# XinArkh/VNect

Measured on AMD Instinct MI355X. Metric: frames/sec, 368x368 3-scale VNect inference, higher is better.
Workload: dtype f32

## Files before the change

include/vnect_abi.h:

```cpp
#ifndef VNECT_ABI_H
#define VNECT_ABI_H
#include <stdint.h>
#ifdef __cplusplus
extern "C" {
#endif

#define VNECT_ABI_VERSION 7
#define VNECT_MAX_SCALES 8
#define VNECT_MAX_STREAMS 4
#define VNECT_BOX 368
#define VNECT_HM 46
#define VNECT_JOINTS 21

enum {
    VNECT_OK = 0,
    VNECT_E_ARG = -1,
    VNECT_E_STATE = -2,
    VNECT_E_HIP = -3,
    VNECT_E_NODEVICE = -4,
    VNECT_E_TIMESTAMP = -5,
    VNECT_E_COMM = -6,
    VNECT_E_TIMEORDER = -7,
    VNECT_E_INTERNAL = -8
};
// ... 197 lines not shown
    double total_ms;
    double net_ms;
    double conv_ms;
    int32_t conv_launches;
    double conv_flops;
    double conv_slot_ms;
    double shader_cycles;
    double shader_ticks;
} vnect_timings;
int vnect_set_profiling(vnect_handle* h, int on);
int vnect_get_timings(vnect_handle* h, vnect_timings* out);
int vnect_reset_timings(vnect_handle* h);

typedef struct vnect_layer_info {
    char name[64];
    int32_t M, N, K;
    int32_t tile_m, tile_n, split_k, workgroups;
    double flops;
    double last_ms;
} vnect_layer_info;
int vnect_get_layer_info(vnect_handle* h, int idx, vnect_layer_info* out);
int vnect_get_batch_layer_info(vnect_handle* h, int idx, vnect_layer_info* out);
int vnect_get_layer_rows(vnect_handle* h, int idx, int batch, int32_t* rows_computed, int32_t* live_rule_stride);
int vnect_get_layer_stamps(vnect_handle* h, int idx, uint64_t* out24);

int vnect_comm_unique_id(void* id128);
int vnect_comm_init(vnect_handle* h, int rank, int nranks, const void* id128);
int vnect_comm_library(char* path_out, int capacity, int32_t* reused_out);
int vnect_comm_p2p_export(vnect_handle* h, void* blob128);
int vnect_comm_p2p_init(vnect_handle* h, int rank, int nranks, const void* blobs);

#ifdef __cplusplus
}
#endif
#endif
```

vnect_amd/_native.py:

```python
import ctypes as C
import os
import subprocess

import numpy as np

_HERE = os.path.dirname(os.path.abspath(__file__))
LIB_PATH = os.environ.get("VNECT_LIB") or os.path.join(_HERE, "lib", "libvnect_hip.so")
_lib = None

MAX_SCALES = 8
OK, E_ARG, E_STATE, E_HIP, E_NODEVICE, E_TIMESTAMP, E_COMM, E_TIMEORDER, E_INTERNAL = 0, -1, -2, -3, -4, -5, -6, -7, -8
ABI_VERSION = 7
MAX_STREAMS = 4
XCHG_RCCL, XCHG_P2P = 0, 1
FP32, BF16, FP32_SPLIT, FP16 = 0, 1, 2, 3


class VnectError(RuntimeError):
    def __init__(self, code, msg):
        super().__init__("libvnect_hip: %s (code %d)" % (msg, code))
        self.code = code


class Config(C.Structure):
# ... 165 lines not shown
    "vnect_forward": (C.c_int, [_H, _f32p, C.c_int, _f32p]),
    "vnect_preprocess": (C.c_int, [_H, _u8p, C.c_int, C.c_int, C.c_int64, _f32p, _f64p, _i32p, _i32p]),
    "vnect_postprocess": (C.c_int, [_H, _f32p, C.c_double, C.c_double, C.c_double, C.c_int32, C.c_int32, _f64p, _f32p]),
    "vnect_infer": (C.c_int, [_H, _u8p, C.c_int, C.c_int, C.c_int64, C.c_double, C.c_double, _f64p, _f32p]),
    "vnect_frame_buffer": (C.c_int, [_H, C.c_int, C.c_int64, C.POINTER(_u8p)]),
    "vnect_upload_frame": (C.c_int, [_H, C.c_int, _u8p, C.c_int, C.c_int, C.c_int64]),
    "vnect_infer_resident": (C.c_int, [_H, C.c_int, C.c_double, C.c_double, _f64p, _f32p]),
    "vnect_submit_resident": (C.c_int, [_H, C.c_int, C.c_double, C.c_double]),
    "vnect_collect": (C.c_int, [_H, _f64p, _f32p]),
    "vnect_submit_stream": (C.c_int, [_H, C.c_int, C.c_int, C.c_double, C.c_double]),
    "vnect_collect_stream": (C.c_int, [_H, _i32p, _f64p, _f32p]),
    "vnect_reset_filters_stream": (C.c_int, [_H, C.c_int]),
    "vnect_set_stream_batch": (C.c_int, [_H, C.c_int]),
    "vnect_submit_streams": (C.c_int, [_H, C.c_int, _i32p, _i32p, _f64p, _f64p]),
    "vnect_get_batch_layer_info": (C.c_int, [_H, C.c_int, C.POINTER(LayerInfo)]),
    "vnect_joint_filter": (C.c_int, [_H, C.c_int, _f64p, C.c_int, C.c_double, _f64p]),
    "vnect_reset_filters": (C.c_int, [_H]),
    "vnect_read_activation": (C.c_int, [_H, C.c_char_p, _f32p, C.c_int64, _i32p]),
    "vnect_set_profiling": (C.c_int, [_H, C.c_int]),
    "vnect_get_timings": (C.c_int, [_H, C.POINTER(Timings)]),
    "vnect_reset_timings": (C.c_int, [_H]),
    "vnect_get_layer_info": (C.c_int, [_H, C.c_int, C.POINTER(LayerInfo)]),
    "vnect_get_layer_rows": (C.c_int, [_H, C.c_int, C.c_int, C.POINTER(C.c_int32), C.POINTER(C.c_int32)]),
    "vnect_get_layer_stamps": (C.c_int, [_H, C.c_int, C.POINTER(C.c_uint64)]),
    "vnect_comm_unique_id": (C.c_int, [C.c_void_p]),
    "vnect_comm_init": (C.c_int, [_H, C.c_int, C.c_int, C.c_void_p]),
    "vnect_comm_library": (C.c_int, [C.c_char_p, C.c_int, _i32p]),
    "vnect_comm_p2p_export": (C.c_int, [_H, C.c_void_p]),
    "vnect_comm_p2p_init": (C.c_int, [_H, C.c_int, C.c_int, C.c_void_p]),
    "vnect_track_begin": (C.c_int, [_H, C.c_int, C.c_int, C.c_int, _i32p]),
    "vnect_submit_tracked": (C.c_int, [_H, C.c_int, C.c_int, C.c_double, C.c_double]),
    "vnect_submit_tracked_pinned": (C.c_int, [_H, C.c_int, C.c_int, C.c_int64, C.c_double, C.c_double]),
    "vnect_collect_tracked": (C.c_int, [_H, _i32p, _f64p, _f32p, _i32p]),
    "vnect_track_box": (C.c_int, [_H, C.c_int, _i32p]),
    "vnect_result_confidence": (C.c_int, [_H, _f64p, _i32p]),
    "vnect_track_policy": (C.c_int, [_H, C.c_int, C.c_double, C.c_int, C.c_int]),
    "vnect_upload_frame_nv12": (C.c_int, [_H, C.c_int, _u8p, C.c_int64, _u8p, C.c_int64, C.c_int, C.c_int]),
    "vnect_upload_frame_nv12_rect": (C.c_int, [_H, C.c_int, _u8p, C.c_int64, _u8p, C.c_int64, C.c_int, C.c_int, _i32p]),
    "vnect_infer_nv12": (C.c_int, [_H, _u8p, C.c_int64, _u8p, C.c_int64, C.c_int, C.c_int, _i32p, C.c_double, C.c_double, _f64p, _f32p]),
    "vnect_preprocess_nv12": (C.c_int, [_H, _u8p, C.c_int64, _u8p, C.c_int64, C.c_int, C.c_int, _i32p, _f32p, _f64p, _i32p, _i32p]),
    "vnect_submit_tracked_pinned_nv12": (C.c_int, [_H, C.c_int, C.c_int, C.c_int64, C.c_int64, C.c_int64, C.c_double, C.c_double]),
    "vnect_read_frame": (C.c_int, [_H, C.c_int, _u8p, C.c_int64, _i32p]),
    "vnect_upload_frame_device": (C.c_int, [_H, C.c_int, C.POINTER(DeviceFrame), C.c_void_p]),
    "vnect_infer_device": (C.c_int, [_H, C.POINTER(DeviceFrame), C.c_void_p, C.c_double, C.c_double, _f64p, _f32p]),
    "vnect_preprocess_device": (C.c_int, [_H, C.POINTER(DeviceFrame), C.c_void_p, _f32p, _f64p, _i32p, _i32p]),
    "vnect_submit_tracked_device": (C.c_int, [_H, C.c_int, C.POINTER(DeviceFrame), C.c_void_p, C.c_double, C.c_double]),
# ... 546 lines not shown
    def reset_timings(self):
        self._ck(lib().vnect_reset_timings(self._h))

    def layer_stamps(self, idx):
        buf = (C.c_uint64 * 24)()
        self._ck(lib().vnect_get_layer_stamps(self._h, idx, buf))
        return list(buf)

    def layers(self):
        return self._layer_list(lib().vnect_get_layer_info)

    def layer_rows(self, batch=False):
        out, i = [], 0
        while True:
            rows, rule = C.c_int32(), C.c_int32()
            rc = lib().vnect_get_layer_rows(self._h, i, int(batch), C.byref(rows), C.byref(rule))
            if rc == E_STATE:
                self._ck(rc)
            if rc:
                return out
            out.append((rows.value, rule.value))
            i += 1

    def _layer_list(self, fn):
        out, i = [], 0
        while True:
            li = LayerInfo()
            rc = fn(self._h, i, C.byref(li))
            if rc == E_STATE:
                self._ck(rc)
            if rc:
                return out
            out.append({k: (getattr(li, k).decode() if k == "name" else getattr(li, k)) for k, _ in LayerInfo._fields_})
            i += 1


def _as_frame(img):
    img = np.asarray(img)
    if img.dtype != np.uint8 or img.ndim != 3 or img.shape[2] != 3:
        raise ValueError("frame must be a uint8 (H, W, 3) BGR array")
    if img.strides[2] != 1 or img.strides[1] != 3 or img.strides[0] < img.shape[1] * 3:
        img = np.ascontiguousarray(img)
    return img


def _as_nv12(nv12):
# ... 134 lines not shown
```

vnect_amd/csrc/conv.hip:

```cpp
#include "kernels.h"

#ifndef X3_DBG
#define X3_DBG 0
#endif
#ifndef VNECT_AB
#define VNECT_AB 0
#endif
#ifndef BF16_NOSTORE
#define BF16_NOSTORE 0
#endif

#include <array>
#include <cstddef>
#include <cstdlib>
#include <type_traits>
#include <utility>

namespace vnect {

typedef float f32x16 __attribute__((ext_vector_type(16)));
typedef float f32x4 __attribute__((ext_vector_type(4)));
typedef __bf16 bf16x8 __attribute__((ext_vector_type(8)));
typedef __bf16 bf16x4 __attribute__((ext_vector_type(4)));
typedef _Float16 f16x8 __attribute__((ext_vector_type(8)));
// ... 58 lines not shown
    *(__attribute__((address_space(1))) h16<BF>*)p = b;
#else
    __hip_atomic_store((unsigned short*)p, __builtin_bit_cast(unsigned short, b), __ATOMIC_RELAXED, __HIP_MEMORY_SCOPE_AGENT);
#endif
}

#if defined(__HIP_DEVICE_COMPILE__)
typedef __amdgpu_buffer_rsrc_t srd_t;
__device__ __forceinline__ srd_t make_srd(const void* base)
{
    return __builtin_amdgcn_make_buffer_rsrc((void*)base, 0, 0x7fffffff, 0x00020000);
}
__device__ __forceinline__ void bload_lds(srd_t r, float* lds, unsigned voff, unsigned soff)
{
    __builtin_amdgcn_raw_ptr_buffer_load_lds(r, (__attribute__((address_space(3))) void*)lds, 16, (int)voff, (int)soff, 0, 0);
}
#else
typedef int srd_t;
__device__ __forceinline__ srd_t make_srd(const void*) { return 0; }
__device__ __forceinline__ void bload_lds(srd_t, float*, unsigned, unsigned) {}
#endif

typedef __attribute__((address_space(3))) unsigned lds_u32;
__device__ __forceinline__ void live_fill(const ConvArgs& a, int M, int Wo, int Ho, unsigned mg_wo, unsigned mg_ho, int m0, int lane, lds_u32* tab)
{
    const int m = m0 + lane;
    const bool ok = m < M;
    const int mm = ok ? m : 0;
    const int t = fdiv(mm, mg_wo, Wo), ox = mm - t * Wo;
    const int sI = fdiv(t, mg_ho, Ho), oy = t - sI * Ho;
    const int pix = (sI * a.OH + oy * a.os) * a.OW + ox * a.os;
    tab[lane] = ok ? (unsigned)(pix * a.ldc) * 4u : 0x80000000u;
}
#if defined(__HIP_DEVICE_COMPILE__)
__device__ __forceinline__ unsigned bload_u32(srd_t r, unsigned voff, unsigned soff) { return __builtin_amdgcn_raw_buffer_load_b32(r, (int)voff, (int)soff, 0); }
__device__ __forceinline__ void bstore_f32(srd_t r, float v, unsigned voff, unsigned soff)
{
    __builtin_amdgcn_raw_buffer_store_b32(__builtin_bit_cast(unsigned, v), r, (int)voff, (int)soff, 16);
}
#else
__device__ __forceinline__ unsigned bload_u32(srd_t, unsigned, unsigned) { return 0; }
__device__ __forceinline__ void bstore_f32(srd_t, float, unsigned, unsigned) {}
#endif
__device__ __forceinline__ void live_load_resid(srd_t rs, const lds_u32* tab, int rb, int cb, int lane, unsigned (&rw)[16])
{
    const unsigned colb = (unsigned)((lane & 31) * 4);
    const lds_u32* lt = tab + rb;
    asm volatile("" ::: "memory");
#pragma unroll
    for (int r = 0; r < 16; r++) rw[r] = bload_u32(rs, lt[(r & 3) + 8 * (r >> 2)] + colb, (unsigned)(cb * 128));
}

constexpr int BONE_N0 = 128, BONE_LS = 68;
__device__ __forceinline__ float bone_len(float x, float y, float z)
{
// ... 559 lines not shown
        auto item_A = [&](const Item& it) __attribute__((always_inline)) {
            tb = __builtin_amdgcn_readfirstlane(it.phase * h.ntaps);
            if constexpr (SPAN) {
                const SpanGeo g = span_geo(it.m0);
                const int slot = wave * 64 + lane;
                const int grow = slot < g.c0 ? g.t0 : g.t0 + 1;
                const int xp = slot < g.c0 ? 2 * g.ox0 + slot : slot - g.c0;
                const int sI = fdiv(grow, h.mg_ho, h.Ho), oy = grow - sI * h.Ho;
                const bool live = slot < g.c0 + g.c1 && grow * h.Wo < h.M;
                a_vo[0] = 0, a_mask[0] = 0;
#pragma unroll
                for (int i = 1; i < ARB; i++) a_vo[i] = 0, a_mask[i] = 0;
                if (live) {
                    const int iy = oy * p.stride, ix = xp;
                    a_vo[0] = (unsigned)(((sI * p.H + iy) * p.W + ix) * p.Cs * ESZ);
                    for (int t2 = 0; t2 < h.ntaps; t2++) {
                        const int y = iy + tap_dy(tb + t2), x = ix + tap_dx(tb + t2);
                        a_mask[0] |= ((unsigned)y < (unsigned)p.H && (unsigned)x < (unsigned)p.W ? 1u : 0u) << t2;
                    }
                }
            }
#pragma unroll
            for (int i = 0; i < (SPAN ? 0 : ARB); i++) {
                const int mraw = it.m0 + srow + 32 * i;
                const bool live = mraw < h.M;
                const int m = live ? mraw : 0;
                const int t = fdiv(m, h.mg_wo, h.Wo), ox = m - t * h.Wo;
                const int s = fdiv(t, h.mg_ho, h.Ho), oy = t - s * h.Ho;
                const int iy = oy * p.stride + (pix && BF ? unit >> 2 : 0);
                const int ix = ox * p.stride + (pix ? (BF ? (unit & 3) * 2 : unit) : 0);
                a_vo[i] = live ? (unsigned)(((s * p.H + iy) * p.W + ix) * p.Cs * ESZ + (pix ? 0 : unit * 16)) : 0u;
                const unsigned vx = (ix >= 1 ? 1u : 0u) | 2u | (ix + 1 < p.W ? 4u : 0u);
                const unsigned m3 = (iy >= 1 ? vx : 0u) | (vx << 3) | (iy + 1 < p.H ? vx << 6 : 0u);
                unsigned mk = a.tapgrid == 1 ? 1u : m3;
                if (a.tapgrid == 0) {
                    mk = 0;
                    for (int t2 = 0; t2 < h.ntaps; t2++) {
                        const int y = iy + tap_dy(tb + t2), x = ix + tap_dx(tb + t2);
                        mk |= ((unsigned)y < (unsigned)p.H && (unsigned)x < (unsigned)p.W ? 1u : 0u) << t2;
                    }
                }
                a_mask[i] = live ? mk : 0u;
            }
            tap = __builtin_amdgcn_readfirstlane(fdiv(it.c0, p.mg_cpt, h.cpt)), cc = __builtin_amdgcn_readfirstlane(it.c0 - tap * h.cpt);
            rem = __builtin_amdgcn_readfirstlane(it.cnt);
            set_tap(tap);
        };
        auto item_B = [&](const Item& it) __attribute__((always_inline)) {
// ... 62 lines not shown
            loads(stage, std::true_type{}, std::true_type{}, 0u);
            advance();
        };
        auto wait_landed = [&](int young) __attribute__((always_inline)) {
            switch (young) {
                case 1: wait_vm<NLD>(); break;
                case 2: wait_vm<2 * NLD>(); break;
                case 3: wait_vm<3 * NLD>(); break;
                case 4: wait_vm<4 * NLD>(); break;
                case 5: wait_vm<5 * NLD>(); break;
                case 6: wait_vm<6 * NLD>(); break;
                case 7: wait_vm<7 * NLD>(); break;
                default: wait_vm<0>(); break;
            }
        };
        TailRegs<BF> T;
        WideRegs<BF> TW;
        const int wm2 = wave & 1, g2 = wave >> 1;
        if constexpr (TAIL && WIDE) wide_load_weights<BF>(a, wave, lane, TW), wide_load_resid<BF>(a, decode(0).m0, wave, lane, TW);
        lds_u32* const ltab = (lds_u32*)smem + (NS - 1) * STAGE + (4 + wave) * 64;
        const bool live = LIVE && a.os != 1;
        if constexpr (TAIL && !WIDE) {
            const int mb2 = decode(0).m0 + wm2 * 32 + 4 * (lane >> 5);
            if (live) {
                if constexpr (LIVE) {
                    live_fill(a, h.M, h.Wo, h.Ho, h.mg_wo, h.mg_ho, decode(0).m0, lane, ltab);
                    const srd_t srdR = make_srd(a.resid);
                    live_load_resid(srdR, ltab, wm2 * 32 + 4 * (lane >> 5), 2 + g2, lane, T.rw[0]);
                    live_load_resid(srdR, ltab, wm2 * 32 + 4 * (lane >> 5), 4 + g2, lane, T.rw[1]);
                }
            } else {
                tail_load_resid<BF>(a, mb2, 2 + g2, lane, T.rw[0]);
                tail_load_resid<BF>(a, mb2, 4 + g2, lane, T.rw[1]);
            }
            tail_load_b<BF>(a, 2 + g2, lane, T.Bf);
        }
        const bool pst = P2 && threadIdx.x == 256 && blockIdx.x == 0;
        if (pst) prof[22] = __builtin_amdgcn_s_memrealtime();
        int nis = 0, istage = 0, g = 0;
        auto put = [&]() __attribute__((always_inline)) {
            issue(istage);
            istage = istage + 1 == NS ? 0 : istage + 1, nis++;
        };
        constexpr bool BFIRST = SINGLE && !X3;
        if constexpr (BFIRST) {
            const Item it = decode(0);
            item_B(it);
            loads(0, std::false_type{}, std::true_type{}, 0u);
            if (G > 1) loads(1, std::false_type{}, std::true_type{}, STEP_B);
            item_A(it);
            if (pst) prof[23] = __builtin_amdgcn_s_memrealtime();
            loads(0, std::true_type{}, std::false_type{}, 0u);
            advance();
            if (G > 1) {
                loads(1, std::true_type{}, std::false_type{}, 0u);
                advance();
            }
            nis = G > 1 ? 2 : 1, istage = nis;
// ... 26 lines not shown
            pw += q1 - q0, pb += q2 - q1, pi += q3 - q2;
        }
        if (pacct) prof[16] = pw, prof[17] = pb, prof[18] = pi;
        if constexpr (TAIL) {
            __builtin_amdgcn_s_barrier();
            if constexpr (WIDE) {
                f32x4 Cq[CHAIN_DEPTH<BF>];
                tail_wide<BF, CHAIN>(a, smem, decode(0).m0, wave, lane, TW, Cq);
                if constexpr (CHAIN) {
                    asm volatile("s_waitcnt lgkmcnt(0)" ::: "memory");
                    __builtin_amdgcn_s_barrier();
                    if constexpr (BF) {
                        if (wide_staged<BF>(a)) wide_write_out(a, smem, decode(0).m0);
                    }
                    chain_gemm<BF>(a, smem, decode(0).m0, wave, lane, Cq);
                } else if constexpr (BF) {
                    if (wide_staged<BF>(a)) {
                        asm volatile("s_waitcnt lgkmcnt(0)" ::: "memory");
                        __builtin_amdgcn_s_barrier();
                        wide_write_out(a, smem, decode(0).m0);
                    }
                }
            } else {
                bool live2 = false;
                if constexpr (LIVE) {
                    int os2;
                    asm volatile("s_load_dword %0, %1, %2\n\ts_waitcnt lgkmcnt(0)" : "=s"(os2) : "s"(__builtin_amdgcn_kernarg_segment_ptr()), "n"(offsetof(ConvArgs, os)) : "memory");
                    live2 = os2 != 1;
                }
                if (live2) live_fill(a, h.M, h.Wo, h.Ho, h.mg_wo, h.mg_ho, decode(0).m0, lane, ltab);
                tail_gemm<BF, 3, true, CHAIN>(a, smem, decode(0).m0, wm2, 2 + g2, 2, lane, T, live2 ? ltab : nullptr);
                if constexpr (CHAIN) chain_narrow<BF>(a, smem, decode(0).m0, wave, lane);
                else if constexpr (BF) {
                    if (tail_staged<BF>(a)) {
                        asm volatile("s_waitcnt lgkmcnt(0)" ::: "memory");
                        __builtin_amdgcn_s_barrier();
                        tail_write_out(a, smem, decode(0).m0);
                    }
                }
            }
        }
        if constexpr (BONE) {
            const Item it0 = decode(0);
            if (it0.n0 <= BONE_N0 && it0.n0 + BN > BONE_N0) {
                __builtin_amdgcn_s_barrier();
                bone_features<BF>(a, smem, it0.m0, it0.phase, tid, h.M, h.Wo, h.Ho, h.mg_wo, h.mg_ho);
            }
        }
        return;
    }

    int fo[4];
#pragma unroll
    for (int q = 0; q < 4; q++) fo[q] = (lane & 31) * 32 + (((2 * q + (lane >> 5)) ^ ((lane >> 1) & 7)) * 4);
// ... 365 lines not shown
                asm volatile("s_waitcnt lgkmcnt(0)" ::: "memory");
                __builtin_amdgcn_s_barrier();
            }
            if constexpr (WIDE) {
                tail_wide<BF, CHAIN>(a, smem, it.m0, 4 + wave, lane, TWc);
                if constexpr (CHAIN) {
                    asm volatile("s_waitcnt lgkmcnt(0)" ::: "memory");
                    __builtin_amdgcn_s_barrier();
                    if constexpr (BF) {
                        if (wide_staged<BF>(a)) wide_write_out(a, smem, it.m0);
                    }
                } else if constexpr (BF) {
                    if (wide_staged<BF>(a)) {
                        asm volatile("s_waitcnt lgkmcnt(0)" ::: "memory");
                        __builtin_amdgcn_s_barrier();
                        wide_write_out(a, smem, it.m0);
                    }
                }
            } else {
                TailRegs<BF> T;
                lds_u32* const ltab = (lds_u32*)smem + (NS - 1) * STAGE + wave * 64;
                const bool live = LIVE && c.os != 1;
                if (live) live_fill(a, h.M, h.Wo, h.Ho, h.mg_wo, h.mg_ho, it.m0, lane, ltab);
                tail_gemm<BF, 1, false, CHAIN>(a, smem, it.m0, wm2, g2, 0, lane, T, live ? ltab : nullptr);
                if constexpr (CHAIN) {
                    asm volatile("s_waitcnt lgkmcnt(0)" ::: "memory");
                    __builtin_amdgcn_s_barrier();
                    tail_write_out(a, smem, it.m0);
                } else if constexpr (BF) {
                    if (tail_staged<BF>(a)) {
                        asm volatile("s_waitcnt lgkmcnt(0)" ::: "memory");
                        __builtin_amdgcn_s_barrier();
                        tail_write_out(a, smem, it.m0);
                    }
                }
            }
            break;
        }
        if constexpr (NACC > 1) {
            asm volatile("s_waitcnt vmcnt(0)" : "+v"(bias), "+v"(sc), "+v"(sh), "+v"(biasx[0]), "+v"(scx[0]), "+v"(shx[0]), "+v"(biasx[NACC - 2]), "+v"(scx[NACC - 2]), "+v"(shx[NACC - 2]));
            const int py = it.phase >> 1, px = it.phase & 1;
            gfloat* const outp = (gfloat*)c.out;
            bool relub[NACC];
#pragma unroll
            for (int b = 0; b < NACC; b++) relub[b] = it.n0 + (wn + b) * 32 < c.relu_cols;
#pragma unroll
            for (int r = 0; r < 16; r++) {
// ... 230 lines not shown
constexpr StreamKernel stream_kernel_at()
{
    constexpr Variant v = variant_at(I);
    static_assert(variant_index(v) == I, "variant_at is the inverse of variant_index: slot I holds the kernel the launcher looks up there");
    if constexpr (variant_exists<BM, BN, KG>(v))
        return {conv_stream_kernel<BM, BN, KG, ring_depth<BM, BN, KG>(v.x3), v.el, v.prof, v.fuse, v.span, v.x3, v.one>, variant_lds<BM, BN, KG>(v.x3)};
    else
        return {nullptr, 0};
}
template <int BM, int BN, int KG, int... I>
constexpr std::array<StreamKernel, sizeof...(I)> stream_kernels(std::integer_sequence<int, I...>)
{
    return {{stream_kernel_at<BM, BN, KG, I>()...}};
}
template <int BM, int BN, int KG>
constexpr auto STREAM_KERNELS = stream_kernels<BM, BN, KG>(std::make_integer_sequence<int, N_VARIANTS>{});

template <int BM, int BN, int KG>
static hipError_t launch_stream(ConvArgs a, hipStream_t st)
{
    if (a.cpt % KG != 0 || a.Npad % BN != 0) return hipErrorInvalidValue;
    a.cpt /= KG;
    int live_grid = 0;
    if (a.live_s != 0) {
        const bool form = BM == 64 && BN == 64 && KG == 1 && a.tail_n == 256 && !a.bf16 && !a.x3 && a.chain_n == 0 && !a.bone;
        if (!form || a.live_s < 2 || !a.resid || a.ldr != a.ldc || a.Nvalid != a.tail_n || a.stride != 1 || a.os != 1 || a.nphase != 1 || a.ksplit != 1 ||
            a.tapgrid != 3 || a.OH != a.Ho || a.OW != a.Wo || a.H != a.Ho || a.W != a.Wo)
            return hipErrorInvalidValue;
        live_grid = ((a.M + BM - 1) / BM) * (a.Npad / BN);
        a.stride = a.os = a.live_s;
        a.Ho = (a.Ho + a.live_s - 1) / a.live_s, a.Wo = (a.Wo + a.live_s - 1) / a.live_s;
        a.M = a.S * a.Ho * a.Wo;
    }
    a.tiles_m = (a.M + BM - 1) / BM, a.tiles_n = a.Npad / BN;
    auto magic = [](int d) { return (unsigned)((0x100000000ull + (unsigned)d - 1) / (unsigned)d); };
    a.mg_wo = magic(a.Wo), a.mg_ho = magic(a.Ho), a.mg_tn = magic(a.tiles_n), a.mg_tm = magic(a.tiles_m);
    a.mg_ks = magic(a.ksplit), a.mg_cpt = magic(a.cpt);
    a.items = a.tiles_m * a.tiles_n * a.nphase * a.ksplit;
    static const int maxwg_env = getenv("VNECT_MAXWG") ? atoi(getenv("VNECT_MAXWG")) : 0;
    const int cus = g_cus;
    const int maxwg = maxwg_env > 0 ? maxwg_env : (KG == 1 && BN <= 64 ? 2 * cus : cus);
    static const bool no_one = getenv("VNECT_NO_ONE") != nullptr, no_big = getenv("VNECT_NO_BIG_GRID") != nullptr;
    const bool plain64 = KG == 1 && BN <= 64 && maxwg_env <= 0 && !no_big && !a.x3 && !a.pixmode;
    const bool big_grid = plain64 && (a.bf16 ? a.items <= 4 * cus : (a.ntaps * a.cpt <= 8 && a.items <= 8 * cus));
    const bool one = a.ksplit == 1 && !no_one && (a.items <= maxwg || big_grid);
    const bool fused = a.tail_n > 0 || a.bone;
    dim3 grid(live_grid ? live_grid : (one || fused) ? a.items : (a.items < maxwg ? a.items : maxwg));
    static const bool detail = getenv("VNECT_PROF_DETAIL") && atoi(getenv("VNECT_PROF_DETAIL")) != 0;
    const int prof = a.prof ? (detail ? 2 : 1) : 0;

    if (a.x3) {
        if (a.bf16 || a.pixmode || a.K % 32) return hipErrorInvalidValue;
        if (a.chain_n != 0) return hipErrorInvalidValue;
    }
    if (a.tail_n > 0) {
        if (a.bone || a.ksplit != 1 || a.nphase != 1 || (a.os != 1 && !live_grid) || !a.tail_w || !a.tail_bias) return hipErrorInvalidValue;
        if constexpr (BN == 128) {
            if (a.Npad != 128 || a.tail_n > 512 ||
                (a.chain_n != 0 && (a.chain_n != 128 || a.tail_n != 512 || !a.chain_w || !a.chain_bias || !a.chain_out || a.chain_ld < 128)))
                return hipErrorInvalidValue;
        } else {
            if (a.Npad != 64 || a.tail_n != 256) return hipErrorInvalidValue;
            if (a.chain_n != 0 && (!a.bf16 || a.chain_n != 64 || !a.chain_w || !a.chain_bias || !a.chain_out || a.chain_ld < 64 || !a.resid ||
                                   a.relu_cols < 256 || a.out_f32 || a.Nvalid != 256 ||
                                   (a.ldc & 7) != 0))
                return hipErrorInvalidValue;
        }
    }
    if (a.bone && (a.ksplit != 1 || a.Npad != 192 || a.ldc < 212)) return hipErrorInvalidValue;
    if constexpr (BN == 96) {
        if (a.bf16 || a.x3 || a.tail_n > 0 || a.resid || a.out2 || a.ksplit != 1 || a.pixmode || (a.relu_cols & 31)) return hipErrorInvalidValue;
    }

    Variant v{};
    v.el = a.f16 ? EL_F16 : a.bf16 ? EL_BF16 : EL_F32;
    v.fuse = a.tail_n > 0 ? (a.chain_n ? 3 : 1) : a.bone ? 2 : 0;
    v.x3 = a.x3 != 0;
    v.span = variant_exists<BM, BN, KG>({EL_F32, 0, 0, true, false, false}) && !v.x3 && v.fuse == 0 && a.pixmode && !a.bf16 && a.ksplit == 1 &&
             a.cpt == 1 && a.Wo >= 64 && a.stride == 2 && getenv("VNECT_NO_SPAN") == nullptr;
// ... 188 lines not shown
```

vnect_amd/csrc/hostplan.h:

```cpp
#pragma once
#include <math.h>
#include <stdint.h>
#include <stdio.h>
#include <stdlib.h>
#include <string.h>

#include <algorithm>
#include <string>
#include <utility>
#include <vector>

#include "axis.h"
#include "tables.h"

namespace vnect {
namespace plan {

inline int cv_round(double v) { return (int)nearbyint(v); }
inline int clipi(int x, int a, int b) { return x >= a ? (x < b ? x : b - 1) : a; }
inline int16_t sat_short(float v)
{
    int r = (int)nearbyintf(v);
    return (int16_t)(r < -32768 ? -32768 : (r > 32767 ? 32767 : r));
}
// ... 408 lines not shown

struct LiveNode {
    int in, resid, out, out2, out3;
    int ntaps, stride;
    int tap00;
    int tail;
};
inline int live_rows_stride(const LiveNode* L, int n, int li, int t_final)
{
    if (li < 0 || li >= n || !L[li].tail || L[li].out < 0 || L[li].out3 >= 0) return 0;
    const int t = L[li].out;
    if (t == t_final) return 0;
    int s = 0;
    for (int j = 0; j < n; j++) {
        if (j == li) continue;
        if (L[j].resid == t) return 0;
        if (L[j].out == t || L[j].out2 == t || L[j].out3 == t) return 0;
        if (L[j].in != t) continue;
        if (L[j].ntaps != 1 || !L[j].tap00 || L[j].stride < 2 || (s && L[j].stride != s)) return 0;
        s = L[j].stride;
    }
    return s;
}
inline int live_dim(int n, int s) { return (n + s - 1) / s; }
inline int live_rows(int S, int Ho, int Wo, int s) { return S * live_dim(Ho, s) * live_dim(Wo, s); }
inline void live_enumeration(int S, int Ho, int Wo, int s, std::vector<int>& pix)
{
    const int Hl = live_dim(Ho, s), Wl = live_dim(Wo, s);
    pix.clear();
    pix.reserve((size_t)S * Ho * Wo);
    for (int j = 0; j < S * Hl * Wl; j++) {
        const int ox = j % Wl, t = j / Wl, oy = t % Hl, im = t / Hl;
        pix.push_back((im * Ho + oy * s) * Wo + ox * s);
    }
    for (int p = 0; p < S * Ho * Wo; p++)
        if ((p % Wo) % s != 0 || ((p / Wo) % Ho) % s != 0) pix.push_back(p);
}
inline int live_wg_tile(int tiles, int grid, int id)
{
    if (id < 0 || id >= grid) return -1;
    const int xcd = id & 7, l = id >> 3, qd = tiles >> 3, rm = tiles & 7;
    const int lo = xcd < rm ? xcd * (qd + 1) : rm * (qd + 1) + (xcd - rm) * qd, cnt = qd + (xcd < rm ? 1 : 0);
    return l < cnt ? lo + l : -1;
}

}
}
```

vnect_amd/csrc/hostplan_capi.cpp:

```cpp
#include <stdint.h>
#include <string.h>

#include <vector>

#include "axis.h"
#include "crop.h"
#include "hostplan.h"

using namespace vnect;

extern "C" {

int hp_resize_u8(const uint8_t* src, int sh, int sw, int ch, double f, uint8_t* dst, int* dh, int* dw)
{
    std::vector<ResizeTab> t(1);
    if (!plan::build_u8_tab(sh, sw, f, &t[0])) return -1;
    *dh = t[0].dh, *dw = t[0].dw;
    if (!dst) return 0;
    for (int y = 0; y < t[0].dh; y++)
        for (int x = 0; x < t[0].dw; x++)
            for (int c = 0; c < ch; c++)
                dst[((size_t)y * t[0].dw + x) * ch + c] =
                    (uint8_t)plan::sample_u8([&](int r, int q) { return (int)src[((size_t)r * sw + q) * ch + c]; }, t[0], y, x);
    return 0;
// ... 248 lines not shown
    memcpy(out, &fp[0], sizeof(FrameParams));
    return status;
}
const char* hp_crop_refusal(int code) { return crop_refusal(code); }
void hp_box_update(const double* j2, int n, int W, int H, int fallback, int32_t* rects)
{
    for (int i = 0; i < n; i++) {
        int r[4];
        box_update(j2 + (size_t)i * NJ * 2, W, H, r);
        if (fallback) box_fallback(W, H, r);
        for (int k = 0; k < 4; k++) rects[(size_t)i * 4 + k] = r[k];
    }
}

int hp_live_rows_stride(const int32_t* nodes, int n, int li, int t_final)
{
    std::vector<plan::LiveNode> L(n > 0 ? n : 0);
    for (int i = 0; i < n; i++) {
        const int32_t* q = nodes + (size_t)i * 9;
        L[i] = {q[0], q[1], q[2], q[3], q[4], q[5], q[6], q[7], q[8]};
    }
    return plan::live_rows_stride(L.data(), n, li, t_final);
}
int hp_live_rows(int S, int Ho, int Wo, int s) { return plan::live_rows(S, Ho, Wo, s); }
void hp_live_enumeration(int S, int Ho, int Wo, int s, int32_t* pix)
{
    std::vector<int> v;
    plan::live_enumeration(S, Ho, Wo, s, v);
    for (size_t i = 0; i < v.size(); i++) pix[i] = v[i];
}
int hp_live_wg_tile(int tiles, int grid, int id) { return plan::live_wg_tile(tiles, grid, id); }

}
```

vnect_amd/csrc/kernels.h:

```cpp
#pragma once
#include <hip/hip_runtime.h>
#include <stdint.h>

#include "tables.h"

namespace vnect {

enum { EL_F32 = 0, EL_BF16 = 1, EL_F16 = 2 };

template <typename T>
struct ElType {
    using type = T;
};
template <typename F>
inline auto with_el(int el, F&& f)
{
    return el == EL_F16 ? f(ElType<_Float16>{}) : el != EL_F32 ? f(ElType<__bf16>{}) : f(ElType<float>{});
}

constexpr int MAX_TAPS = 16;
constexpr int ARG_SLABS_MAX = 32;
constexpr int PROF_WGS = 512;
constexpr int PROF_SLOTS = 28;

// ... 24 lines not shown
    int pixmode;
    int bf16;
    int out_f32;
    int f16;
    int tiles_m, tiles_n;
    int items;
    unsigned mg_ks, mg_cpt;
    unsigned mg_wo, mg_ho, mg_tn, mg_tm;
    long long w_phase_stride;
    int tap_bias;
    unsigned long long dy_pack, dx_pack;
    int tapgrid;
    const float* tail_w;
    const float* tail_bias;
    int x3;
    int bone;
    int tail_n;
    const float* chain_w;
    const float* chain_bias;
    float* chain_out;
    int chain_n;
    int chain_ld;
    int live_s;
};

struct ReduceArgs {
    const float* ws;
    long long slab_pix;
    const float* bias;
    const float* scale;
    const float* shift;
    const float* resid;
    float* out;
    long long npix;
    int Npad, Nvalid, ldc, ldr, ksplit, relu_cols;
    int bf16, out_f32, f16;
};

#if defined(__HIP_DEVICE_COMPILE__)
template <typename V>
__device__ __forceinline__ void store_wt(V* p, V v)
{
    static_assert(sizeof(V) == 16 || sizeof(V) == 8, "one dwordx4 / dwordx2 store");
    if constexpr (sizeof(V) == 16) asm volatile("global_store_dwordx4 %0, %1, off sc1\n\ts_nop 2" ::"v"(p), "v"(v) : "memory");
    else asm volatile("global_store_dwordx2 %0, %1, off sc1" ::"v"(p), "v"(v) : "memory");
}
// ... 215 lines not shown
```

vnect_amd/csrc/rt_abi.cpp:

```cpp
#include "runtime.h"

namespace vnect {
namespace rt {
thread_local std::string g_create_error = "";
}
}

static int preprocess_slot0(vnect_handle* h, float* batch_out, double* scaler, int32_t* offset_x, int32_t* offset_y)
{
    FrameParams fp;
    int rc;
    if ((rc = squarify_params(h, h->slots[0].H, h->slots[0].W, &fp))) return rc;
    if ((rc = sync_geometry(h, fp))) return rc;
    if ((rc = run_pre(h, slot_dyn(h, 0, 0.0, 0.0), false, true))) return rc;
    if (batch_out) {
        const long long npix = (long long)h->Snet * BOX * BOX;
        HIPCK(h, launch_strip4to3(h->tensors[h->t_input4].d, h->in3, npix, h->el(), h->st));
        HIPCK(h, hipMemcpyAsync(batch_out, h->in3, npix * 3 * sizeof(float), hipMemcpyDeviceToHost, h->st));
    }
    HIPCK(h, hipStreamSynchronize(h->st));
    if (scaler) *scaler = fp.scaler;
    if (offset_x) *offset_x = fp.offx;
    if (offset_y) *offset_y = fp.offy;
    return VNECT_OK;
// ... 633 lines not shown
    });
}

static int rows_computed(const std::vector<Layer>& layers, int idx, int32_t* rows)
{
    if (!rows || idx < 0 || idx >= (int)layers.size()) return VNECT_E_ARG;
    const Layer& L = layers[idx];
    *rows = L.op != OP_CONV ? 0 : L.a.live_s ? plan::live_rows(L.a.S, L.a.Ho, L.a.Wo, L.a.live_s) : L.a.M * L.a.nphase;
    return VNECT_OK;
}

int vnect_get_layer_rows(vnect_handle* h, int idx, int batch, int32_t* rows_computed_out, int32_t* live_rule_stride)
{
    return guarded(&h, [&]() -> int {
        if (!h) return VNECT_E_ARG;
        if (batch && h->bplans.empty()) return fail(h, VNECT_E_STATE, "vnect_get_layer_rows: no batched plan (vnect_set_stream_batch(h, 2), then vnect_finalize)");
        const std::vector<Layer>& layers = batch ? h->bplans[0]->layers : h->layers;
        const int rc = rows_computed(layers, idx, rows_computed_out);
        if (rc == VNECT_OK && live_rule_stride) *live_rule_stride = live_rows_of(layers, idx, h->t_out);
        return rc;
    });
}

int vnect_set_stream_batch(vnect_handle* h, int n)
{
    return guarded(&h, [&]() -> int {
        if (!h) return VNECT_E_ARG;
        if (h->finalized || h->pre_only) return fail(h, VNECT_E_STATE, "vnect_set_stream_batch after vnect_finalize or on a preprocess_only handle");
        if (h->sharded) return fail(h, VNECT_E_ARG, "vnect_set_stream_batch: a pyramid-sharded handle serves one stream");
        if (n < 1 || n > 2) return fail(h, VNECT_E_ARG, "vnect_set_stream_batch: n must be 1 or 2");
        if (2 * h->Snet > VNECT_MAX_SCALES && n == 2) return fail(h, VNECT_E_ARG, "vnect_set_stream_batch: 2 x num_scales exceeds VNECT_MAX_SCALES");
        if (h->people && n == 2) return fail(h, VNECT_E_ARG, "vnect_set_stream_batch: not together with vnect_set_people");
        h->stream_batch = n;
        return VNECT_OK;
    });
}

int vnect_submit_streams(vnect_handle* h, int n, const int32_t* streams, const int32_t* slots, const double* t2d, const double* t3d)
{
    return guarded(&h, [&]() -> int {
        if (!h) return VNECT_E_ARG;
        if (!streams || !slots || !t2d || !t3d) return fail(h, VNECT_E_ARG, "vnect_submit_streams: bad argument");
        if (!h->finalized) return fail(h, VNECT_E_STATE, "inference before vnect_finalize");
        if (n != 1 && n != 2) return fail(h, VNECT_E_ARG, "vnect_submit_streams: n must be 1 or 2");
        HIPCK(h, hipSetDevice(h->cfg.device));
        if (n == 1) {
// ... 504 lines not shown
```

vnect_amd/csrc/rt_plan.cpp:

```cpp
#include "runtime.h"

namespace vnect {
namespace rt {

static int upload_weights(vnect_handle* h, float** dst, const std::vector<float>& v)
{
    if (!h->bf16) return upload(h, dst, v);
    std::vector<uint16_t> b;
    plan::to_16(v, h->f16, b);
    uint16_t* p = nullptr;
    int rc = upload(h, &p, b);
    *dst = (float*)p;
    return rc;
}

static int upload_layer_weights(vnect_handle* h, Layer& L, const std::vector<float>& wp)
{
    ConvArgs& a = L.a;
    a.x3 = h->x3 && !h->bf16 && L.BM == 64 && L.BN * L.KG == 64 && !a.pixmode && a.K % 32 == 0 && !getenv("VNECT_NO_X3");
    if (!a.x3) return upload_weights(h, &L.w, wp);
    std::vector<uint16_t> pl;
    plan::pack_split3(wp, std::max(a.nphase, 1), a.Npad, a.K, pl);
    uint16_t* p = nullptr;
    int rc = upload(h, &p, pl);
// ... 269 lines not shown
    a.tail_w = dw2, a.tail_bias = db2, a.tail_n = cout;
    if (chain_out) *chain_out = -1;
    const bool chain_wide = wide && cout == 512 && (h->bf16 || getenv("VNECT_FORCE_CHAIN"));
    const bool chain_narrow = narrow && !wide && cout == 256 && h->bf16 && resid >= 0;
    if ((chain_wide || chain_narrow) && relu2 && !chain_scope.empty() && chain_out && !getenv("VNECT_NO_CHAIN")) {
        const int cn = chain_wide ? 128 : 64;
        const HostArray* Wn = get_w(h, chain_scope + "/weights", {1, 1, cout, cn});
        const HostArray* Bn = Wn ? get_w(h, chain_scope + "/biases", {cn}) : nullptr;
        if (!Bn) return -1;
        std::vector<float> w3, b3(Bn->d.begin(), Bn->d.end());
        plan::pack_tail(Wn->d.data(), cout, cn, h->bf16, w3);
        float *dw3 = nullptr, *db3 = nullptr;
        if (upload_weights(h, &dw3, w3) || upload(h, &db3, b3)) return -1;
        L.out3 = add_tensor(h, chain_scope, tin.S, ho, wo, cn, cn);
        a.chain_w = dw3, a.chain_bias = db3, a.chain_n = cn, a.chain_ld = cn;
        L.name += ">" + chain_scope;
        L.flops += 2.0 * a.M * (double)cout * cn;
        *chain_out = L.out3;
    }
    h->layers.push_back(L);
    return L.out;
}

int live_rows_of(const std::vector<Layer>& layers, int li, int t_out)
{
    std::vector<plan::LiveNode> n(layers.size());
    for (size_t i = 0; i < layers.size(); i++) {
        const Layer& L = layers[i];
        const bool cv = L.op == OP_CONV;
        n[i] = {L.in, L.resid, L.out, L.out2, L.out3, cv ? L.a.ntaps * L.a.nphase : 0, cv ? L.a.stride : 1,
                cv && L.dy[0] == 0 && L.dx[0] == 0 && !L.a.pixmode, cv && L.a.tail_n > 0};
    }
    return plan::live_rows_stride(n.data(), (int)n.size(), li, t_out);
}
static void mark_live_rows(vnect_handle* h)
{
    if (getenv("VNECT_NO_LIVE_ROWS")) return;
    if (h->keep_activations && !(h->keep_fused && getenv("VNECT_FORCE_LIVE_ROWS"))) return;
    for (size_t li = 0; li < h->layers.size(); li++) {
        Layer& L = h->layers[li];
        ConvArgs& a = L.a;
        if (L.op != OP_CONV || a.tail_n != 256 || L.BM != 64 || L.BN != 64 || a.bf16 || a.x3 || a.chain_n || L.resid < 0) continue;
        const int s = live_rows_of(h->layers, (int)li, h->t_out);
        if (s < 2) continue;
        a.live_s = s;
        L.flops *= (double)plan::live_rows(a.S, a.Ho, a.Wo, s) / a.M;
    }
}

bool plan_writes(const Plan* p, int t)
{
    if (t == p->t_input4) return true;
    for (int li = 0; li < (int)p->layers.size(); li++) {
        if (p->stem_mode && (li == p->l_conv1 || (p->stem_pair && li == p->l_pool1))) continue;
        const Layer& L = p->layers[li];
// ... 266 lines not shown
            Layer Bn;
            Bn.op = OP_BONE, Bn.name = "res5c_bone_length", Bn.in = feat, Bn.out = feat;
            h->layers.push_back(Bn);
        }
    }
    {
        const HostArray* Wk = get_w(h, "res5c_branch2c/kernel", {1, 1, 128, 84});
        if (!Wk) return VNECT_E_ARG;
        HostArray z;
        z.d.assign(84, 0.f), z.shape = {84};
        h->weights["res5c_branch2c/weights"] = *Wk;
        h->weights["res5c_branch2c/biases"] = z;
        bool fits = false;
        h->t_out = add_conv_tail(h, "res5c_branch2b", "res5c_branch2c", feat, -1, "res5c_branch2c", 128, 84, &fits, false);
        if (!fits) {
            const int hd = conv("res5c_branch2b", feat, 3, 1, 128, true);
            h->t_out = hd < 0 ? -1 : conv("res5c_branch2c", hd, 1, 1, 84, false);
        }
        h->weights.erase("res5c_branch2c/weights"), h->weights.erase("res5c_branch2c/biases");
        NEED(h->t_out);
    }
#undef NEED
    mark_live_rows(h);
    if (!h->keep_activations) {
        int rc = alloc_arena(h);
        if (rc) return rc;
    } else {
        for (Tensor& t : h->tensors) {
            char* p = nullptr;
            int rc = dev_alloc(h, &p, padded(t));
            if (rc) return rc;
            t.d = (float*)p;
            HIPCK(h, hipMemset(t.d, 0, padded(t)));
        }
    }
    int rcw = alloc_workspace(h);
    if (rcw) return rcw;
    HIPCK(h, hipDeviceSynchronize());
    h->conv_flops = 0, h->conv_launches = 0;
    for (Layer& L : h->layers) {
        if (L.op != OP_CONV) continue;
        ConvArgs& a = L.a;
        a.f16 = a.bf16 && h->f16;
        bind_activations(h, L);
        {
            const int esz = a.bf16 ? 2 : 4, nt = a.nphase * a.ntaps;
// ... 119 lines not shown
```

vnect_amd/csrc/runtime.h:

```cpp
#pragma once
#include <dlfcn.h>
#include <link.h>
#include <unistd.h>
#include <math.h>
#include <stdio.h>
#include <stdlib.h>
#include <string.h>
#include <time.h>
#include <stddef.h>

#include <algorithm>
#include <map>
#include <mutex>
#include <string>
#include <vector>

#include "../../include/vnect_abi.h"
#include "crop.h"
#include "hostplan.h"
#include "ingest.h"
#include "kernels.h"
#include "orient.h"
#include "overlay.h"
#include "preview.h"
// ... 322 lines not shown
    h->param_cur += need, h->param_left -= need;
    return VNECT_OK;
}

template <typename T>
int upload(vnect_handle* h, T** dst, const std::vector<T>& v)
{
    int rc = param_alloc(h, dst, v.size());
    if (rc) return rc;
    HIPCK(h, hipMemcpy(*dst, v.data(), v.size() * sizeof(T), hipMemcpyHostToDevice));
    return VNECT_OK;
}

int build_scale_tables(vnect_handle* h);
int build_up_table(vnect_handle* h);
int squarify_params(vnect_handle* h, int H, int W, FrameParams* fp);
int add_tensor(vnect_handle* h, const std::string& name, int S, int H, int W, int C, int Cs, bool force_f32 = false);
int finalize_impl(vnect_handle* h);
int build_plans(vnect_handle* h);
void destroy_plan(Plan* p);
void destroy_plans(vnect_handle* h);
bool plan_writes(const Plan* p, int tensor);
int live_rows_of(const std::vector<Layer>& layers, int li, int t_out);

int run_network(Plan* p, bool timed, bool stem_done = false);
int sync_geometry(Plan* p, const FrameParams& fp, int which = 0);
int run_pre(Plan* p, const FrameDyn& dyn, bool timed = false, bool want_batch = false);
int run_argmax(Plan* p);
int run_joints(Plan* p, const FrameDyn& dyn, JointsOut* out, ConfOut* conf, int stream = 0, const FrameParams* fp = nullptr, double* conf_dev = nullptr);
int run_post(Plan* p, const FrameDyn& dyn, JointsOut* out, ConfOut* conf, int stream = 0, const FrameParams* fp = nullptr, double* conf_dev = nullptr);
void deliver_confidence(vnect_handle* h, int ring, bool tracked);
int check_time(vnect_handle* h, const Stream& s, double t2d, double t3d);
void commit_time(Stream& s, double t2d, double t3d);
int reset_filters_impl(vnect_handle* h, int stream = -1);
void roctx_load();
int build_graph(Plan* p);
enum FrameWhere {
    SRC_SLOT,
    SRC_PINNED_BGR,
    SRC_NV12,
    SRC_DEVICE
};
struct PinnedBgr {
    const uint8_t* data;
    long long stride;
    const uint8_t* end;
// ... 84 lines not shown
```

Baseline: 1171.

## Skip dead residual rows and use half-size tiles for small live-row convs

Adds a dead-row stride to conv tail layers whose output is read only by strided live-row consumers, so the tail writes only the rows those consumers will read. Also adds a half-tile mode (32-row M tiles) for live-row convs whose reduced M fits within the CU count, which spreads the few remaining rows across more workgroups. This cuts store traffic and improves occupancy on small layers, at the cost of more complex bit-packed os flags and extra branching in the tail kernels.

After: 1176 (median of 6 runs). About the same (+0.4%).

```diff
diff --git a/include/vnect_abi.h b/include/vnect_abi.h
--- a/include/vnect_abi.h
+++ b/include/vnect_abi.h
@@ -243,6 +243,7 @@
 int vnect_get_layer_info(vnect_handle* h, int idx, vnect_layer_info* out);
 int vnect_get_batch_layer_info(vnect_handle* h, int idx, vnect_layer_info* out);
 int vnect_get_layer_rows(vnect_handle* h, int idx, int batch, int32_t* rows_computed, int32_t* live_rule_stride);
+int vnect_get_layer_traffic_rows(vnect_handle* h, int idx, int batch, int32_t* rows_stored, int32_t* dead_rule_stride);
 int vnect_get_layer_stamps(vnect_handle* h, int idx, uint64_t* out24);
 
 int vnect_comm_unique_id(void* id128);
diff --git a/vnect_amd/_native.py b/vnect_amd/_native.py
--- a/vnect_amd/_native.py
+++ b/vnect_amd/_native.py
@@ -211,6 +211,7 @@
     "vnect_reset_timings": (C.c_int, [_H]),
     "vnect_get_layer_info": (C.c_int, [_H, C.c_int, C.POINTER(LayerInfo)]),
     "vnect_get_layer_rows": (C.c_int, [_H, C.c_int, C.c_int, C.POINTER(C.c_int32), C.POINTER(C.c_int32)]),
+    "vnect_get_layer_traffic_rows": (C.c_int, [_H, C.c_int, C.c_int, C.POINTER(C.c_int32), C.POINTER(C.c_int32)]),
     "vnect_get_layer_stamps": (C.c_int, [_H, C.c_int, C.POINTER(C.c_uint64)]),
     "vnect_comm_unique_id": (C.c_int, [C.c_void_p]),
     "vnect_comm_init": (C.c_int, [_H, C.c_int, C.c_int, C.c_void_p]),
@@ -803,6 +804,18 @@
             out.append((rows.value, rule.value))
             i += 1
 
+    def layer_traffic_rows(self, batch=False):
+        out, i = [], 0
+        while True:
+            rows, rule = C.c_int32(), C.c_int32()
+            rc = lib().vnect_get_layer_traffic_rows(self._h, i, int(batch), C.byref(rows), C.byref(rule))
+            if rc == E_STATE:
+                self._ck(rc)
+            if rc:
+                return out
+            out.append((rows.value, rule.value))
+            i += 1
+
     def _layer_list(self, fn):
         out, i = [], 0
         while True:
diff --git a/vnect_amd/csrc/conv.hip b/vnect_amd/csrc/conv.hip
--- a/vnect_amd/csrc/conv.hip
+++ b/vnect_amd/csrc/conv.hip
@@ -104,15 +104,20 @@
 #endif
 
 typedef __attribute__((address_space(3))) unsigned lds_u32;
+constexpr int LIVE_OS_MASK = 0xff, LIVE_HALF = 0x200, LIVE_DEAD_SHIFT = 16;
 __device__ __forceinline__ void live_fill(const ConvArgs& a, int M, int Wo, int Ho, unsigned mg_wo, unsigned mg_ho, int m0, int lane, lds_u32* tab)
 {
-    const int m = m0 + lane;
-    const bool ok = m < M;
+    const int osf = a.os, os = osf & LIVE_OS_MASK;
+    const bool half = (osf & LIVE_HALF) != 0;
+    const int m = (half ? m0 >> 1 : m0) + lane;
+    const bool ok = m < M && !(half && lane >= 32);
     const int mm = ok ? m : 0;
     const int t = fdiv(mm, mg_wo, Wo), ox = mm - t * Wo;
     const int sI = fdiv(t, mg_ho, Ho), oy = t - sI * Ho;
-    const int pix = (sI * a.OH + oy * a.os) * a.OW + ox * a.os;
-    tab[lane] = ok ? (unsigned)(pix * a.ldc) * 4u : 0x80000000u;
+    const int pix = (sI * a.OH + oy * os) * a.OW + ox * os;
+    const int dmask = (int)((unsigned)osf >> LIVE_DEAD_SHIFT);
+    const bool keep = ok && ((oy | ox) & dmask) == 0;
+    tab[lane] = keep ? (unsigned)(pix * a.ldc) * 4u : 0x80000000u;
 }
 #if defined(__HIP_DEVICE_COMPILE__)
 __device__ __forceinline__ unsigned bload_u32(srd_t r, unsigned voff, unsigned soff) { return __builtin_amdgcn_raw_buffer_load_b32(r, (int)voff, (int)soff, 0); }
@@ -718,8 +723,13 @@
             }
 #pragma unroll
             for (int i = 0; i < (SPAN ? 0 : ARB); i++) {
-                const int mraw = it.m0 + srow + 32 * i;
-                const bool live = mraw < h.M;
+                int mraw = it.m0 + srow + 32 * i;
+                bool live = mraw < h.M;
+                if constexpr (LIVE) {
+                    const bool half = (a.os & LIVE_HALF) != 0;
+                    mraw = half ? (it.m0 >> 1) + srow : mraw;
+                    live = mraw < h.M && !(half && i == 1);
+                }
                 const int m = live ? mraw : 0;
                 const int t = fdiv(m, h.mg_wo, h.Wo), ox = m - t * h.Wo;
                 const int s = fdiv(t, h.mg_ho, h.Ho), oy = t - s * h.Ho;
@@ -828,18 +838,24 @@
         const bool live = LIVE && a.os != 1;
         if constexpr (TAIL && !WIDE) {
             const int mb2 = decode(0).m0 + wm2 * 32 + 4 * (lane >> 5);
+            int cbf = 2 + g2;
             if (live) {
                 if constexpr (LIVE) {
                     live_fill(a, h.M, h.Wo, h.Ho, h.mg_wo, h.mg_ho, decode(0).m0, lane, ltab);
                     const srd_t srdR = make_srd(a.resid);
-                    live_load_resid(srdR, ltab, wm2 * 32 + 4 * (lane >> 5), 2 + g2, lane, T.rw[0]);
-                    live_load_resid(srdR, ltab, wm2 * 32 + 4 * (lane >> 5), 4 + g2, lane, T.rw[1]);
+                    if ((a.os & LIVE_HALF) != 0) {
+                        cbf = 4 + wave;
+                        live_load_resid(srdR, ltab, 4 * (lane >> 5), cbf, lane, T.rw[0]);
+                    } else {
+                        live_load_resid(srdR, ltab, wm2 * 32 + 4 * (lane >> 5), 2 + g2, lane, T.rw[0]);
+                        live_load_resid(srdR, ltab, wm2 * 32 + 4 * (lane >> 5), 4 + g2, lane, T.rw[1]);
+                    }
                 }
             } else {
                 tail_load_resid<BF>(a, mb2, 2 + g2, lane, T.rw[0]);
                 tail_load_resid<BF>(a, mb2, 4 + g2, lane, T.rw[1]);
             }
-            tail_load_b<BF>(a, 2 + g2, lane, T.Bf);
+            tail_load_b<BF>(a, cbf, lane, T.Bf);
         }
         const bool pst = P2 && threadIdx.x == 256 && blockIdx.x == 0;
         if (pst) prof[22] = __builtin_amdgcn_s_memrealtime();
@@ -912,14 +928,15 @@
                     }
                 }
             } else {
-                bool live2 = false;
+                bool live2 = false, half2 = false;
                 if constexpr (LIVE) {
                     int os2;
                     asm volatile("s_load_dword %0, %1, %2\n\ts_waitcnt lgkmcnt(0)" : "=s"(os2) : "s"(__builtin_amdgcn_kernarg_segment_ptr()), "n"(offsetof(ConvArgs, os)) : "memory");
-                    live2 = os2 != 1;
+                    live2 = os2 != 1, half2 = (os2 & LIVE_HALF) != 0;
                 }
                 if (live2) live_fill(a, h.M, h.Wo, h.Ho, h.mg_wo, h.mg_ho, decode(0).m0, lane, ltab);
-                tail_gemm<BF, 3, true, CHAIN>(a, smem, decode(0).m0, wm2, 2 + g2, 2, lane, T, live2 ? ltab : nullptr);
+                if (LIVE && half2) tail_gemm<BF, 1, true, CHAIN>(a, smem, decode(0).m0, 0, 4 + wave, 0, lane, T, ltab);
+                else tail_gemm<BF, 3, true, CHAIN>(a, smem, decode(0).m0, wm2, 2 + g2, 2, lane, T, live2 ? ltab : nullptr);
                 if constexpr (CHAIN) chain_narrow<BF>(a, smem, decode(0).m0, wave, lane);
                 else if constexpr (BF) {
                     if (tail_staged<BF>(a)) {
@@ -1331,7 +1348,8 @@
                 lds_u32* const ltab = (lds_u32*)smem + (NS - 1) * STAGE + wave * 64;
                 const bool live = LIVE && c.os != 1;
                 if (live) live_fill(a, h.M, h.Wo, h.Ho, h.mg_wo, h.mg_ho, it.m0, lane, ltab);
-                tail_gemm<BF, 1, false, CHAIN>(a, smem, it.m0, wm2, g2, 0, lane, T, live ? ltab : nullptr);
+                const bool half = LIVE && (c.os & LIVE_HALF) != 0;
+                tail_gemm<BF, 1, false, CHAIN>(a, smem, it.m0, half ? 0 : wm2, half ? wave : g2, 0, lane, T, live ? ltab : nullptr);
                 if constexpr (CHAIN) {
                     asm volatile("s_waitcnt lgkmcnt(0)" ::: "memory");
                     __builtin_amdgcn_s_barrier();
@@ -1608,17 +1626,29 @@
     if (a.cpt % KG != 0 || a.Npad % BN != 0) return hipErrorInvalidValue;
     a.cpt /= KG;
     int live_grid = 0;
+    bool live_half = false;
     if (a.live_s != 0) {
         const bool form = BM == 64 && BN == 64 && KG == 1 && a.tail_n == 256 && !a.bf16 && !a.x3 && a.chain_n == 0 && !a.bone;
-        if (!form || a.live_s < 2 || !a.resid || a.ldr != a.ldc || a.Nvalid != a.tail_n || a.stride != 1 || a.os != 1 || a.nphase != 1 || a.ksplit != 1 ||
+        if (!form || a.live_s < 2 || a.live_s > LIVE_OS_MASK || !a.resid || a.ldr != a.ldc || a.Nvalid != a.tail_n || a.stride != 1 || a.os != 1 || a.nphase != 1 || a.ksplit != 1 ||
             a.tapgrid != 3 || a.OH != a.Ho || a.OW != a.Wo || a.H != a.Ho || a.W != a.Wo)
             return hipErrorInvalidValue;
         live_grid = ((a.M + BM - 1) / BM) * (a.Npad / BN);
         a.stride = a.os = a.live_s;
         a.Ho = (a.Ho + a.live_s - 1) / a.live_s, a.Wo = (a.Wo + a.live_s - 1) / a.live_s;
         a.M = a.S * a.Ho * a.Wo;
-    }
-    a.tiles_m = (a.M + BM - 1) / BM, a.tiles_n = a.Npad / BN;
+        static const bool no_half = getenv("VNECT_NO_HALF_TILES") != nullptr;
+        const int tiles32 = (a.M + 31) / 32;
+        live_half = !no_half && tiles32 <= g_cus && tiles32 <= live_grid;
+        if (live_half) a.os |= LIVE_HALF;
+    }
+    if (a.dead_s != 0) {
+        const bool form = BM == 64 && BN == 64 && KG == 1 && a.tail_n == 256 && !a.bf16 && !a.x3 && a.chain_n == 0 && !a.bone;
+        if (!form || a.live_s != 0 || a.dead_s < 2 || a.dead_s > 0x4000 || (a.dead_s & (a.dead_s - 1)) != 0 || !a.resid || a.ldr != a.ldc || a.Nvalid != a.tail_n || a.stride != 1 ||
+            a.os != 1 || a.nphase != 1 || a.ksplit != 1 || a.tapgrid != 3 || a.OH != a.Ho || a.OW != a.Wo || a.H != a.Ho || a.W != a.Wo)
+            return hipErrorInvalidValue;
+        a.os = 1 | ((a.dead_s - 1) << LIVE_DEAD_SHIFT);
+    }
+    a.tiles_m = live_half ? (a.M + 31) / 32 : (a.M + BM - 1) / BM, a.tiles_n = a.Npad / BN;
     auto magic = [](int d) { return (unsigned)((0x100000000ull + (unsigned)d - 1) / (unsigned)d); };
     a.mg_wo = magic(a.Wo), a.mg_ho = magic(a.Ho), a.mg_tn = magic(a.tiles_n), a.mg_tm = magic(a.tiles_m);
     a.mg_ks = magic(a.ksplit), a.mg_cpt = magic(a.cpt);
@@ -1640,7 +1670,7 @@
         if (a.chain_n != 0) return hipErrorInvalidValue;
     }
     if (a.tail_n > 0) {
-        if (a.bone || a.ksplit != 1 || a.nphase != 1 || (a.os != 1 && !live_grid) || !a.tail_w || !a.tail_bias) return hipErrorInvalidValue;
+        if (a.bone || a.ksplit != 1 || a.nphase != 1 || (a.os != 1 && !live_grid && !a.dead_s) || !a.tail_w || !a.tail_bias) return hipErrorInvalidValue;
         if constexpr (BN == 128) {
             if (a.Npad != 128 || a.tail_n > 512 ||
                 (a.chain_n != 0 && (a.chain_n != 128 || a.tail_n != 512 || !a.chain_w || !a.chain_bias || !a.chain_out || a.chain_ld < 128)))
diff --git a/vnect_amd/csrc/hostplan.h b/vnect_amd/csrc/hostplan.h
--- a/vnect_amd/csrc/hostplan.h
+++ b/vnect_amd/csrc/hostplan.h
@@ -454,6 +454,23 @@
     }
     return s;
 }
+inline int dead_rows_stride(const LiveNode* L, int n, int li, int t_final)
+{
+    if (li < 0 || li >= n || !L[li].tail || L[li].out < 0 || L[li].out3 >= 0) return 0;
+    const int t = L[li].out;
+    if (t == t_final) return 0;
+    int s = 0;
+    for (int j = 0; j < n; j++) {
+        if (j == li) continue;
+        if (L[j].out == t || L[j].out2 == t || L[j].out3 == t) return 0;
+        if (L[j].in == t) return 0;
+        if (L[j].resid != t) continue;
+        const int sj = live_rows_stride(L, n, j, t_final);
+        if (sj < 2 || (s && sj != s)) return 0;
+        s = sj;
+    }
+    return s;
+}
 inline int live_dim(int n, int s) { return (n + s - 1) / s; }
 inline int live_rows(int S, int Ho, int Wo, int s) { return S * live_dim(Ho, s) * live_dim(Wo, s); }
 inline void live_enumeration(int S, int Ho, int Wo, int s, std::vector<int>& pix)
@@ -475,6 +492,11 @@
     const int lo = xcd < rm ? xcd * (qd + 1) : rm * (qd + 1) + (xcd - rm) * qd, cnt = qd + (xcd < rm ? 1 : 0);
     return l < cnt ? lo + l : -1;
 }
-
-}
-}
+inline int live_wg_half_tile(int tiles32, int grid, int id)
+{
+    if (tiles32 > grid) return -1;
+    return live_wg_tile(tiles32, grid, id);
+}
+
+}
+}
diff --git a/vnect_amd/csrc/hostplan_capi.cpp b/vnect_amd/csrc/hostplan_capi.cpp
--- a/vnect_amd/csrc/hostplan_capi.cpp
+++ b/vnect_amd/csrc/hostplan_capi.cpp
@@ -294,6 +294,15 @@
     }
     return plan::live_rows_stride(L.data(), n, li, t_final);
 }
+int hp_dead_rows_stride(const int32_t* nodes, int n, int li, int t_final)
+{
+    std::vector<plan::LiveNode> L(n > 0 ? n : 0);
+    for (int i = 0; i < n; i++) {
+        const int32_t* q = nodes + (size_t)i * 9;
+        L[i] = {q[0], q[1], q[2], q[3], q[4], q[5], q[6], q[7], q[8]};
+    }
+    return plan::dead_rows_stride(L.data(), n, li, t_final);
+}
 int hp_live_rows(int S, int Ho, int Wo, int s) { return plan::live_rows(S, Ho, Wo, s); }
 void hp_live_enumeration(int S, int Ho, int Wo, int s, int32_t* pix)
 {
@@ -302,5 +311,6 @@
     for (size_t i = 0; i < v.size(); i++) pix[i] = v[i];
 }
 int hp_live_wg_tile(int tiles, int grid, int id) { return plan::live_wg_tile(tiles, grid, id); }
-
-}
+int hp_live_wg_half_tile(int tiles32, int grid, int id) { return plan::live_wg_half_tile(tiles32, grid, id); }
+
+}
diff --git a/vnect_amd/csrc/kernels.h b/vnect_amd/csrc/kernels.h
--- a/vnect_amd/csrc/kernels.h
+++ b/vnect_amd/csrc/kernels.h
@@ -70,6 +70,7 @@
     int chain_n;
     int chain_ld;
     int live_s;
+    int dead_s;
 };
 
 struct ReduceArgs {
diff --git a/vnect_amd/csrc/rt_abi.cpp b/vnect_amd/csrc/rt_abi.cpp
--- a/vnect_amd/csrc/rt_abi.cpp
+++ b/vnect_amd/csrc/rt_abi.cpp
@@ -679,6 +679,21 @@
     });
 }
 
+int vnect_get_layer_traffic_rows(vnect_handle* h, int idx, int batch, int32_t* rows_stored, int32_t* dead_rule_stride)
+{
+    return guarded(&h, [&]() -> int {
+        if (!h) return VNECT_E_ARG;
+        if (batch && h->bplans.empty()) return fail(h, VNECT_E_STATE, "vnect_get_layer_traffic_rows: no batched plan (vnect_set_stream_batch(h, 2), then vnect_finalize)");
+        const std::vector<Layer>& layers = batch ? h->bplans[0]->layers : h->layers;
+        const int rc = rows_computed(layers, idx, rows_stored);
+        if (rc != VNECT_OK) return rc;
+        const Layer& L = layers[idx];
+        if (L.op == OP_CONV && L.a.dead_s) *rows_stored = plan::live_rows(L.a.S, L.a.Ho, L.a.Wo, L.a.dead_s);
+        if (dead_rule_stride) *dead_rule_stride = dead_rows_of(layers, idx, h->t_out);
+        return rc;
+    });
+}
+
 int vnect_set_stream_batch(vnect_handle* h, int n)
 {
     return guarded(&h, [&]() -> int {
diff --git a/vnect_amd/csrc/rt_plan.cpp b/vnect_amd/csrc/rt_plan.cpp
--- a/vnect_amd/csrc/rt_plan.cpp
+++ b/vnect_amd/csrc/rt_plan.cpp
@@ -315,7 +315,7 @@
     return L.out;
 }
 
-int live_rows_of(const std::vector<Layer>& layers, int li, int t_out)
+static std::vector<plan::LiveNode> live_nodes(const std::vector<Layer>& layers)
 {
     std::vector<plan::LiveNode> n(layers.size());
     for (size_t i = 0; i < layers.size(); i++) {
@@ -324,6 +324,32 @@
         n[i] = {L.in, L.resid, L.out, L.out2, L.out3, cv ? L.a.ntaps * L.a.nphase : 0, cv ? L.a.stride : 1,
                 cv && L.dy[0] == 0 && L.dx[0] == 0 && !L.a.pixmode, cv && L.a.tail_n > 0};
     }
+    return n;
+}
+int dead_rows_of(const std::vector<Layer>& layers, int li, int t_out)
+{
+    const std::vector<plan::LiveNode> n = live_nodes(layers);
+    return plan::dead_rows_stride(n.data(), (int)n.size(), li, t_out);
+}
+static void mark_dead_rows(vnect_handle* h)
+{
+    if (getenv("VNECT_NO_DEAD_ROWS")) return;
+    if (h->keep_activations && !(h->keep_fused && getenv("VNECT_FORCE_DEAD_ROWS"))) return;
+    for (size_t li = 0; li < h->layers.size(); li++) {
+        Layer& L = h->layers[li];
+        ConvArgs& a = L.a;
+        if (L.op != OP_CONV || a.tail_n != 256 || L.BM != 64 || L.BN != 64 || a.bf16 || a.x3 || a.chain_n || L.resid < 0 || a.live_s) continue;
+        const int s = dead_rows_of(h->layers, (int)li, h->t_out);
+        if (s < 2 || (s & (s - 1)) != 0) continue;
+        bool readers_live = true;
+        for (const Layer& R : h->layers)
+            if (R.resid == L.out && !(R.op == OP_CONV && R.a.live_s == s)) readers_live = false;
+        if (readers_live) a.dead_s = s;
+    }
+}
+int live_rows_of(const std::vector<Layer>& layers, int li, int t_out)
+{
+    const std::vector<plan::LiveNode> n = live_nodes(layers);
     return plan::live_rows_stride(n.data(), (int)n.size(), li, t_out);
 }
 static void mark_live_rows(vnect_handle* h)
@@ -636,6 +662,7 @@
     }
 #undef NEED
     mark_live_rows(h);
+    mark_dead_rows(h);
     if (!h->keep_activations) {
         int rc = alloc_arena(h);
         if (rc) return rc;
diff --git a/vnect_amd/csrc/runtime.h b/vnect_amd/csrc/runtime.h
--- a/vnect_amd/csrc/runtime.h
+++ b/vnect_amd/csrc/runtime.h
@@ -368,6 +368,7 @@
 void destroy_plans(vnect_handle* h);
 bool plan_writes(const Plan* p, int tensor);
 int live_rows_of(const std::vector<Layer>& layers, int li, int t_out);
+int dead_rows_of(const std::vector<Layer>& layers, int li, int t_out);
 
 int run_network(Plan* p, bool timed, bool stem_done = false);
 int sync_geometry(Plan* p, const FrameParams& fp, int which = 0);
```
